# microhh/rte-rrtmgp-cpp

Hardware: AMD Instinct MI355X
Metric: columns/sec (LW+SW full solve, 140 lay x 256 gpt) (higher is better)
Workload: dtype f64; 1 GPU; C4 synthetic 16384 columns/GPU (16384 in total) x 140 layers x 256 g-points, LW+SW clear-sky, RCEMIP profile, synthetic k-distribution (real shapes); columns_per_gpu=16384, columns_total=16384, nlay=140, ngpt=256, flux_mode=broadband (do_broadband solvers, g-point sums on chip), columns_sorted=False, parallelism=columns sharded x1, all-gather of broadband fluxes

## Files before the change

rte-rrtmgp-cpp_amd/csrc/rrx_common.h:

```cpp
#ifndef RRX_COMMON_H
#define RRX_COMMON_H

#include <hip/hip_runtime.h>
#include <cfloat>
#include <cstdlib>
#include <cmath>
#include <string>
#include <vector>
#include <stdexcept>
#include <type_traits>

typedef signed char Bool;

namespace rrx
{
    struct Tuning
    {
        int lw_variant = 0;
        int sw_variant = 0;
        int bb_min_groups = 512;
        int bb_gsplit = 0;
        int sync_waves = 1;
        int go_share = 1;
        int go_window = 1;
    };
    Tuning& tuning();

    void set_error(const std::string& msg);
    int check_launch(const char* what);

    constexpr int WAVE = 64;

    template<typename F> struct Lim;
    template<> struct Lim<double>
    {
        __host__ __device__ static constexpr double eps() { return DBL_EPSILON; }
        __host__ __device__ static constexpr double tiny() { return DBL_MIN; }
        __host__ __device__ static constexpr double k_min() { return 1.e-12; }
    };
    template<> struct Lim<float>
    {
        __host__ __device__ static constexpr float eps() { return FLT_EPSILON; }
        __host__ __device__ static constexpr float tiny() { return FLT_MIN; }
        __host__ __device__ static constexpr float k_min() { return 1.e-4f; }
    };

    __device__ __forceinline__ float shfl(const float v, const int src_lane) { return __shfl(v, src_lane, WAVE); }
    __device__ __forceinline__ double shfl(const double v, const int src_lane) { return __shfl(v, src_lane, WAVE); }

#ifndef RRX_NT_LOADS
#define RRX_NT_LOADS 0
#endif
#ifndef RRX_NT_STORES
#define RRX_NT_STORES 0
#endif
    template<typename F, int V> struct Vec { F v[V]; };

    template<typename F, int V>
    __device__ __forceinline__ Vec<F,V> load_cols(const F* __restrict__ p)
    {
        Vec<F,V> r;
        if constexpr (V == 1)
        {
#if RRX_NT_LOADS
            r.v[0] = __builtin_nontemporal_load(p);
#else
            r.v[0] = p[0];
#endif
        }
        else
        {
            typedef F vecT __attribute__((ext_vector_type(V)));
#if RRX_NT_LOADS
            const vecT t = __builtin_nontemporal_load(reinterpret_cast<const vecT*>(p));
#else
            const vecT t = *reinterpret_cast<const vecT*>(p);
#endif
            #pragma unroll
            for (int i=0; i<V; ++i) r.v[i] = t[i];
        }
        return r;
    }

    template<typename F, int V>
    __device__ __forceinline__ void store_cols(F* __restrict__ p, const Vec<F,V>& r)
    {
        if constexpr (V == 1)
        {
#if RRX_NT_STORES
            __builtin_nontemporal_store(r.v[0], p);
#else
            p[0] = r.v[0];
#endif
        }
        else
        {
            typedef F vecT __attribute__((ext_vector_type(V)));
            vecT t;
            #pragma unroll
            for (int i=0; i<V; ++i) t[i] = r.v[i];
#if RRX_NT_STORES
            __builtin_nontemporal_store(t, reinterpret_cast<vecT*>(p));
#else
            *reinterpret_cast<vecT*>(p) = t;
#endif
        }
    }

    template<typename F>
    __device__ __forceinline__ void add_rounded(F& acc, const F x)
    {
        #pragma clang fp contract(off)
        acc = acc + x;
    }

    __device__ __forceinline__ double fast_rcp(const double x)
    {
        double r = __builtin_amdgcn_rcp(x);
        double e = fma(-x, r, 1.0); r = fma(r, e, r);
        e = fma(-x, r, 1.0); r = fma(r, e, r);
        return r;
    }
#ifndef RRX_F32_IEEE_RCP
    __device__ __forceinline__ float fast_rcp(const float x)
    {
        float r = __builtin_amdgcn_rcpf(x);
        const float e = fmaf(-x, r, 1.0f); r = fmaf(r, e, r);
        return r;
    }
#else
    __device__ __forceinline__ float fast_rcp(const float x) { return 1.0f / x; }
#endif

    __device__ __forceinline__ double exp_neg(const double x)
    {
        const double n = __builtin_rint(x * 0x1.71547652b82fep+0);
        double r = fma(n, -0x1.62e42f0000000p-1, x);
        r = fma(n, -0x1.df473de6af279p-26, r);
        double p = 0x1.af389ecfc4b9cp-26;
        p = fma(p, r, 0x1.28917c89a43a7p-22); p = fma(p, r, 0x1.71de0db2f6b19p-19); p = fma(p, r, 0x1.a019b9149a41cp-16);
        p = fma(p, r, 0x1.a01a01a7c2efep-13); p = fma(p, r, 0x1.6c16c17889ef1p-10); p = fma(p, r, 0x1.11111111109b5p-7);
        p = fma(p, r, 0x1.5555555553d68p-5); p = fma(p, r, 0x1.5555555555556p-3); p = fma(p, r, 0x1.0000000000001p-1);
        const double t = fma(r*r, p, r);
        return __builtin_amdgcn_ldexp(t + 1.0, (int)n);
    }
    static __device__ const double exp2_64_table[64] = {
        0x1.0000000000000p+0, 0x1.02c9a3e778061p+0, 0x1.059b0d3158574p+0, 0x1.0874518759bc8p+0, 0x1.0b5586cf9890fp+0, 0x1.0e3ec32d3d1a2p+0,
        0x1.11301d0125b51p+0, 0x1.1429aaea92de0p+0, 0x1.172b83c7d517bp+0, 0x1.1a35beb6fcb75p+0, 0x1.1d4873168b9aap+0, 0x1.2063b88628cd6p+0,
        0x1.2387a6e756238p+0, 0x1.26b4565e27cddp+0, 0x1.29e9df51fdee1p+0, 0x1.2d285a6e4030bp+0, 0x1.306fe0a31b715p+0, 0x1.33c08b26416ffp+0,
        0x1.371a7373aa9cbp+0, 0x1.3a7db34e59ff7p+0, 0x1.3dea64c123422p+0, 0x1.4160a21f72e2ap+0, 0x1.44e086061892dp+0, 0x1.486a2b5c13cd0p+0,
        0x1.4bfdad5362a27p+0, 0x1.4f9b2769d2ca7p+0, 0x1.5342b569d4f82p+0, 0x1.56f4736b527dap+0, 0x1.5ab07dd485429p+0, 0x1.5e76f15ad2148p+0,
        0x1.6247eb03a5585p+0, 0x1.6623882552225p+0, 0x1.6a09e667f3bcdp+0, 0x1.6dfb23c651a2fp+0, 0x1.71f75e8ec5f74p+0, 0x1.75feb564267c9p+0,
        0x1.7a11473eb0187p+0, 0x1.7e2f336cf4e62p+0, 0x1.82589994cce13p+0, 0x1.868d99b4492edp+0, 0x1.8ace5422aa0dbp+0, 0x1.8f1ae99157736p+0,
        0x1.93737b0cdc5e5p+0, 0x1.97d829fde4e50p+0, 0x1.9c49182a3f090p+0, 0x1.a0c667b5de565p+0, 0x1.a5503b23e255dp+0, 0x1.a9e6b5579fdbfp+0,
        0x1.ae89f995ad3adp+0, 0x1.b33a2b84f15fbp+0, 0x1.b7f76f2fb5e47p+0, 0x1.bcc1e904bc1d2p+0, 0x1.c199bdd85529cp+0, 0x1.c67f12e57d14bp+0,
        0x1.cb720dcef9069p+0, 0x1.d072d4a07897cp+0, 0x1.d5818dcfba487p+0, 0x1.da9e603db3285p+0, 0x1.dfc97337b9b5fp+0, 0x1.e502ee78b3ff6p+0,
        0x1.ea4afa2a490dap+0, 0x1.efa1bee615a27p+0, 0x1.f50765b6e4540p+0, 0x1.fa7c1819e90d8p+0};
    __device__ __forceinline__ void exp_table_fill(double* lds_table)
    {
        if (threadIdx.x < 64) lds_table[threadIdx.x] = exp2_64_table[threadIdx.x];
    }
    __device__ __forceinline__ double exp_neg(const double x, const double* lds_table)
    {
        const double magic = 0x1.8p+52;
        const double t = fma(x, 0x1.71547652b82fep+6, magic);
        const double nf = t - magic;
// ... 204 lines not shown
```

rte-rrtmgp-cpp_amd/csrc/rrx_solver_lw.hip:

```cpp
#include "rrx_common.h"
#include "rrx_hip.h"

#pragma clang fp contract(fast)

namespace
{
using namespace rrx;

constexpr int CL = 8;
constexpr int LL = 8;

template<typename F, int V, int K, bool JAC, bool ACC>
__global__ void __launch_bounds__(256, 2)
lw_noscat_scan_kernel(
        const int ncol, const int nlay, const int ngpt, const int top_at_1, const int imu,
        const F* __restrict__ secants, const F* __restrict__ weights,
        const F* __restrict__ tau, const F* __restrict__ lay_source, const F* __restrict__ lev_source,
        const F* __restrict__ sfc_emis, const F* __restrict__ sfc_src, const F* __restrict__ inc_flux,
        F* __restrict__ flux_up, F* __restrict__ flux_dn,
        const F* __restrict__ sfc_src_jac, F* __restrict__ flux_up_jac, const int sync_waves)
{
    constexpr int W = 2;
    const int lane = threadIdx.x & 63;
    const int wave = threadIdx.x >> 6;
// ... 179 lines not shown
    {
        F dn[V];
        #pragma unroll
        for (int v=0; v<V; ++v) dn[v] = dn_in[v];
        #pragma unroll
        for (int j=0; j<K; ++j)
        {
            Vec<F,V> o;
            #pragma unroll
            for (int v=0; v<V; ++v) { o.v[v] = scale * dn[v]; dn[v] = tr[j][v]*dn[v] + sdn[j][v]; }
            put(flux_dn, j, o);
        }
    }
    {
        F up[V], jc[V];
        #pragma unroll
        for (int v=0; v<V; ++v) { up[v] = up_in[v]; jc[v] = JAC ? jac_in[v] : F(0.); }
        #pragma unroll
        for (int j=K-1; j>=0; --j)
        {
            Vec<F,V> o, oj;
            #pragma unroll
            for (int v=0; v<V; ++v)
            {
                up[v] = tr[j][v]*up[v] + sup[j][v];
                o.v[v] = scale * up[v];
                if constexpr (JAC) { jc[v] = tr[j][v]*jc[v]; oj.v[v] = scale * jc[v]; }
            }
            put(flux_up, j, o);
            if constexpr (JAC) put(flux_up_jac, j, oj);
        }
    }
    }
}


#ifndef RRX_LW_LACC
#define RRX_LW_LACC 1
#endif
#ifndef RRX_LW_EXP_TABLE
#define RRX_LW_EXP_TABLE 1
#endif
#ifndef RRX_LW_TIMING
#define RRX_LW_TIMING 0
#endif
#if RRX_LW_TIMING
__device__ unsigned long long g_lw_clk[16][8];
#define RRX_LW_T(k) { const unsigned long long t_ = __builtin_readcyclecounter(); lw_acc[k] += t_ - lw_t; lw_t = t_; }
#else
#define RRX_LW_T(k)
#endif
#ifndef RRX_LW_LACC32
#define RRX_LW_LACC32 1
#endif
#ifndef RRX_LW_EV
#define RRX_LW_EV 1
#endif
#ifndef RRX_LW_F32_WAVES
#define RRX_LW_F32_WAVES 2
#endif
template<typename F, int V, int K, int W, int CLT, bool LITE, bool GS = false, int EV = RRX_LW_EV, int NW = (W > 4 ? W : 4), bool BND = false,
         bool JAC = false, bool MU = false, bool OPT = false>
__global__ void __launch_bounds__(64*NW, (NW > W) ? RRX_LW_F32_WAVES : (NW > 4 ? 1 : 2))
lw_noscat_bb_kernel(
        const int ncol, const int nlay, const int ngpt, const int top_at_1,
        const F* __restrict__ secants, const F* __restrict__ weights,
        const F* __restrict__ tau, const F* __restrict__ lay_source , const F* __restrict__ lev_source,
        const F* __restrict__ blay, const F* __restrict__ blev, const int* __restrict__ gpoint_bands,
        const F* __restrict__ sfc_emis, const F* __restrict__ sfc_src, const F* __restrict__ inc_flux,
        F* __restrict__ flux_up, F* __restrict__ flux_dn, const int gper, const size_t part_stride,
        const int* __restrict__ band_lims, const F* __restrict__ sfc_src_jac = nullptr, F* __restrict__ flux_up_jac = nullptr,
        const int nmus = 1, const F* __restrict__ opt_fit = nullptr, F* __restrict__ secants_out = nullptr)
{
    static_assert(!(GS && BND), "a by-band launch is its own g-point split");
    static_assert(!(JAC && BND), "no by-band Jacobian");
    static_assert(!MU || (LITE && !BND), "several angles: Planck-lite inputs, no by-band form");
    static_assert(!OPT || (LITE && !BND), "optimal angles: Planck-lite inputs, no by-band form");
    static_assert(!(OPT && MU), "optimal angles are one quadrature angle");
    const int g_lo = BND ? max(band_lims[2*blockIdx.y] - 1, 0) : (GS ? blockIdx.y*gper : 0);
    const int g_hi = BND ? min(band_lims[2*blockIdx.y+1], ngpt) : (GS ? min(ngpt, g_lo + gper) : ngpt);
    if constexpr (GS || BND) { flux_up += blockIdx.y*part_stride; flux_dn += blockIdx.y*part_stride; }
    if constexpr (GS && JAC) flux_up_jac += blockIdx.y*part_stride;
    constexpr int CL = CLT, LL = 64/CLT;
    const int tid = threadIdx.x, lane = tid & 63, wave = tid >> 6;
    const int cl = lane & (CL-1), ll = lane / CL;
    const int h = wave % W, w0 = wave - h;
    const int bx = ((NW/W)*CL*V*sizeof(F) < 128) ? xcd_contiguous(blockIdx.x, gridDim.x) : int(blockIdx.x);
    const int wave_col0 = (bx*(NW/W) + wave/W) * (CL*V);
    __shared__ F xch[4*V][NW][CL];
    __shared__ F xsum[OPT ? V : 1][NW][CL];
    __shared__ F lds_b[LITE ? (2*K+1)*V : 1][64*NW];
    constexpr bool ETAB = sizeof(F) == 8 && RRX_LW_EXP_TABLE;
    __shared__ F lds_etab[ETAB ? 64 : 1];
    if constexpr (ETAB) { exp_table_fill(lds_etab); __syncthreads(); }
    int icol = wave_col0 + cl*V;
    const bool active = icol < ncol;
    if (!active) icol = (wave_col0 < ncol) ? wave_col0 : 0;
    const bool writer = active && wave_col0 < ncol;
    const int nlev = nlay + 1;
    const size_t ncl = size_t(ncol);
    const int t0 = (h*LL + ll)*K;
    const F pi = F(3.14159265358979323846);
    const F tau_thres = sqrt(sqrt(Lim<F>::eps()));

    constexpr bool LACC = RRX_LW_LACC && ((sizeof(F) == 8 && V == 1) || (sizeof(F) == 4 && V == 2 && RRX_LW_LACC32));
    __shared__ F lds_acc[LACC ? 2*K*V : 1][64*NW];
    F acc_up[LACC ? 1 : K][V], acc_dn[LACC ? 1 : K][V];
    #pragma unroll
    for (int j=0; j<K; ++j)
        #pragma unroll
        for (int v=0; v<V; ++v)
        {
            if constexpr (LACC) { lds_acc[j*V+v][tid] = F(0.); lds_acc[(K+j)*V+v][tid] = F(0.); }
            else { acc_up[j][v] = F(0.); acc_dn[j][v] = F(0.); }
        }
    F acc_jc[JAC ? K : 1][V];
    if constexpr (JAC)
    {
        #pragma unroll
        for (int j=0; j<K; ++j)
            #pragma unroll
            for (int v=0; v<V; ++v) acc_jc[j][v] = F(0.);
    }

    auto lay_off = [&](const int j) -> unsigned
    {
        const int sc = min(max(t0 + j, 0), nlay-1);
        return unsigned(top_at_1 ? sc : nlay-1-sc)*unsigned(ncol) + unsigned(icol);
    };
    auto lev_off = [&](const int j) -> unsigned
    {
        const int tc = min(t0 + j, nlay);
        return unsigned(top_at_1 ? tc : nlay-tc)*unsigned(ncol) + unsigned(icol);
    };

    struct Loads { Vec<F,V> a0[K], a1[K], a2[LITE ? 1 : K], x_next, x_prev, emis, ssrc, D, inc; };
    auto issue = [&](const int g, Loads& L, Vec<F,V>& J)
    {
        const F* __restrict__ t_g = tau + size_t(g)*ncl*nlay;
        const F* __restrict__ l_g = lay_source + size_t(g)*ncl*nlay;
        #pragma unroll
        for (int j=0; j<K; ++j) { const unsigned o = lay_off(j); L.a0[j] = load_cols<F,V>(t_g + o); L.a1[j] = load_cols<F,V>(l_g + o); }
        if constexpr (!LITE)
        {
            const F* __restrict__ v_g = lev_source + size_t(g)*ncl*nlev;
            #pragma unroll
            for (int j=0; j<K; ++j) L.a2[j] = load_cols<F,V>(v_g + lev_off(j));
            L.x_next = load_cols<F,V>(v_g + lev_off(K));
        }
        else
        {
            L.x_next = load_cols<F,V>(l_g + lay_off(K));
            L.x_prev = load_cols<F,V>(l_g + lay_off(-1));
        }
        const size_t sfc = size_t(g)*ncl + icol;
        L.emis = load_cols<F,V>(sfc_emis + sfc); L.ssrc = load_cols<F,V>(sfc_src + sfc);
        if constexpr (!MU && !OPT) L.D = load_cols<F,V>(secants + sfc);
        if (inc_flux != nullptr) L.inc = load_cols<F,V>(inc_flux + sfc);
        if constexpr (JAC) J = load_cols<F,V>(sfc_src_jac + sfc);
    };

    Loads nxt;
    Vec<F,V> jnxt, jcur;
    if (!BND || g_lo < g_hi) issue(g_lo, nxt, jnxt);
    int cur_bnd = -1;
    const F wgt = weights[0];
    const F scale = pi * wgt;
    Vec<F,V> d_next, c_emis, c_ssrc, c_inc;
    F scale_mu;
    if constexpr (MU) d_next = load_cols<F,V>(secants + size_t(g_lo)*ncl + icol);
    F fit1 = F(0.), fit2 = F(0.);

#if RRX_LW_TIMING
    unsigned long long lw_acc[8] = {0, 0, 0, 0, 0, 0, 0, 0}, lw_t = __builtin_readcyclecounter();
#endif
    for (int igpt=g_lo; igpt<g_hi; ++igpt)
    {
    RRX_LW_T(7)
    std::conditional_t<MU, Loads&, Loads> cur = nxt;
    if constexpr (JAC) jcur = jnxt;
    if constexpr (MU) { c_emis = cur.emis; c_ssrc = cur.ssrc; c_inc = cur.inc; }

    if constexpr (LITE)
    {
        const int ib = gpoint_bands[igpt] - 1;
        if (ib != cur_bnd)
        {
            cur_bnd = ib;
            const F* __restrict__ bl = blay + size_t(ib)*ncl*nlay;
            const F* __restrict__ bv = blev + size_t(ib)*ncl*nlev;
            #pragma unroll
            for (int j=0; j<K; ++j)
            {
                const Vec<F,V> x = load_cols<F,V>(bl + lay_off(j));
                #pragma unroll
                for (int v=0; v<V; ++v) lds_b[j*V+v][tid] = x.v[v];
            }
            #pragma unroll
            for (int j=0; j<=K; ++j)
            {
                const Vec<F,V> x = load_cols<F,V>(bv + lev_off(j));
                #pragma unroll
                for (int v=0; v<V; ++v) lds_b[(K+j)*V+v][tid] = x.v[v];
            }
            if constexpr (OPT) { fit1 = opt_fit[2*ib]; fit2 = opt_fit[2*ib+1]; }
        }
    }

    if constexpr (OPT)
    {
        F s[V];
        #pragma unroll
        for (int v=0; v<V; ++v) s[v] = F(0.);
        #pragma unroll
        for (int j=0; j<K; ++j)
        {
            const bool valid = (t0 + j) < nlay;
            #pragma unroll
            for (int v=0; v<V; ++v) s[v] += valid ? cur.a0[j].v[v] : F(0.);
        }
        #pragma unroll
        for (int d=1; d<LL; d<<=1)
            #pragma unroll
            for (int v=0; v<V; ++v) s[v] += shfl(s[v], lane ^ (d*CL));
        if (ll == 0)
        {
            #pragma unroll
            for (int v=0; v<V; ++v) xsum[v][wave][cl] = s[v];
        }
        RRX_LW_T(4)
        __syncthreads();
        #pragma unroll
        for (int v=0; v<V; ++v)
        {
            F t = F(0.);
            #pragma unroll
            for (int w=0; w<W; ++w) t += xsum[v][w0+w][cl];
            F e;
            if constexpr (ETAB) e = exp_neg(-t, lds_etab); else e = exp_neg(-t);
            cur.D.v[v] = fit1*e + fit2;
// ... 18 lines not shown
    do
    {
    if constexpr (MU)
    {
        cur.D = d_next;
        scale_mu = pi * weights[imu];
        const bool last = imu == nmus-1;
        d_next = load_cols<F,V>(secants + (size_t(last ? 0 : imu + 1)*ngpt + (last ? min(igpt + 1, g_hi - 1) : igpt))*ncl + icol);
        #pragma unroll
        for (int j=0; j<K; ++j)
            #pragma unroll
            for (int v=0; v<V; ++v) asm volatile("" : "+v"(cur.a1[j].v[v]));
        #pragma unroll
        for (int v=0; v<V; ++v) asm volatile("" : "+v"(cur.x_prev.v[v]), "+v"(cur.x_next.v[v]));
    }
    F tr[K][V], sdn[K][V], sup[K][V];
    F A[V], Bdn[V], Bup[V], lva[V];
    #pragma unroll
    for (int v=0; v<V; ++v) { A[v] = F(1.); Bdn[v] = F(0.); Bup[v] = F(0.); lva[v] = level_src(0, v); }
    #pragma unroll
    for (int j=0; j<K; ++j)
    {
        const bool valid = (t0 + j) < nlay;
        #pragma unroll
        for (int v=0; v<V; ++v)
        {
            F tvj = cur.a0[j].v[v];
            const int e = j*V + v - EV*V;
            if (e >= 0) asm volatile("" : "+v"(tvj) : "v"(sup[e / V][e % V]));
            const F lvb = level_src(j+1, v);
            F lsj = cur.a1[j].v[v];
            if constexpr (LITE) lsj *= lds_b[j*V+v][tid];
            const F tau_loc = (valid ? tvj : F(0.)) * cur.D.v[v];
            F trans;
            if constexpr (ETAB) trans = exp_neg(-tau_loc, lds_etab); else trans = exp_neg(-tau_loc);
            const F fact = tau_loc > tau_thres ? (F(1.) - trans) * fast_rcp(tau_loc) - trans
                                               : tau_loc * (F(.5) + tau_loc * (F(-1./3.) + tau_loc * F(1./8.)));
            const F omt = F(1.) - trans;
            const F s_dn = omt * lvb + F(2.) * fact * (lsj - lvb);
            const F s_up = omt * lva[v] + F(2.) * fact * (lsj - lva[v]);
            lva[v] = lvb;
            tr[j][v] = trans; sdn[j][v] = s_dn; sup[j][v] = s_up;
            Bdn[v] = tr[j][v]*Bdn[v] + sdn[j][v];
            Bup[v] += A[v]*sup[j][v];
            A[v] *= tr[j][v];
        }
    }

    RRX_LW_T(0)
    F dn_in[V], up_in[V], jc_in[V];
    #pragma unroll
    for (int v=0; v<V; ++v)
    {
        F a = A[v], b = Bdn[v];
        #pragma unroll
        for (int d=1; d<LL; d<<=1)
        {
            const F a2 = shfl(a, lane - d*CL), b2 = shfl(b, lane - d*CL);
            if (ll >= d) { b = a*b2 + b; a = a*a2; }
        }
        F xa = F(1.), xb = F(0.);
        if (ll == LL-1) { xch[4*v+0][wave][cl] = a; xch[4*v+1][wave][cl] = b; }
        RRX_LW_T(1)
        __syncthreads();
        RRX_LW_T(6)
        if (v == 0) if (!MU || imu == nmus-1)
        {
            __builtin_amdgcn_sched_barrier(0);
            issue(min(igpt + 1, g_hi - 1), nxt, jnxt);
            __builtin_amdgcn_sched_barrier(0);
        }
        F fa = F(1.), fb = F(0.);
        #pragma unroll
        for (int w=0; w<W; ++w)
        {
            const F oa = xch[4*v+0][w0+w][cl], ob = xch[4*v+1][w0+w][cl];
            if (w == h) { xa = fa; xb = fb; }
            fb = oa*fb + ob; fa = oa*fa;
        }
        if (h > 0) { b = a*xb + b; a = a*xa; }
        F ae = shfl(a, lane - CL), be = shfl(b, lane - CL);
        if (ll == 0) { ae = xa; be = xb; }
        const F dn_top = (inc_flux != nullptr) ? (MU ? c_inc : cur.inc).v[v] / pi : F(0.);
        dn_in[v] = ae*dn_top + be;
        const F dn_sfc = fa*dn_top + fb;
        const F up_sfc = dn_sfc * (F(1.) - (MU ? c_emis : cur.emis).v[v]) + (MU ? c_emis : cur.emis).v[v] * (MU ? c_ssrc : cur.ssrc).v[v];

        a = A[v]; b = Bup[v];
        #pragma unroll
        for (int d=1; d<LL; d<<=1)
        {
            const F a2 = shfl(a, lane + d*CL), b2 = shfl(b, lane + d*CL);
            if (ll + d < LL) { b = a*b2 + b; a = a*a2; }
        }
        xa = F(1.); xb = F(0.);
        if (ll == 0) { xch[4*v+2][wave][cl] = a; xch[4*v+3][wave][cl] = b; }
        RRX_LW_T(2)
        __syncthreads();
        RRX_LW_T(6)
        #pragma unroll
        for (int w=W-1; w>=1; --w)
            if (w > h) { const F oa = xch[4*v+2][w0+w][cl], ob = xch[4*v+3][w0+w][cl]; xb = oa*xb + ob; xa = oa*xa; }
        if (h < W-1) { b = a*xb + b; a = a*xa; }
        ae = shfl(a, lane + CL); be = shfl(b, lane + CL);
        if (ll == LL-1) { ae = xa; be = xb; }
        up_in[v] = ae*up_sfc + be;
        if constexpr (JAC) jc_in[v] = ae * (MU ? c_emis : cur.emis).v[v] * jcur.v[v];
    }

    #pragma unroll
    for (int v=0; v<V; ++v)
    {
        F dn = dn_in[v];
        #pragma unroll
        for (int j=0; j<K; ++j)
        {
            if constexpr (LACC) { F a = lds_acc[(K+j)*V+v][tid]; add_rounded(a, (MU ? scale_mu : scale)*dn); lds_acc[(K+j)*V+v][tid] = a; }
            else add_rounded(acc_dn[j][v], (MU ? scale_mu : scale)*dn);
            dn = tr[j][v]*dn + sdn[j][v];
        }
        F up = up_in[v];
        #pragma unroll
        for (int j=K-1; j>=0; --j)
        {
            up = tr[j][v]*up + sup[j][v];
            if constexpr (LACC) { F a = lds_acc[j*V+v][tid]; add_rounded(a, (MU ? scale_mu : scale)*up); lds_acc[j*V+v][tid] = a; }
            else add_rounded(acc_up[j][v], (MU ? scale_mu : scale)*up);
        }
        if constexpr (JAC)
        {
            F jc = jc_in[v];
            #pragma unroll
            for (int j=K-1; j>=0; --j) { jc = tr[j][v]*jc; add_rounded(acc_jc[j][v], (MU ? scale_mu : scale)*jc); }
        }
    }
    RRX_LW_T(3)
    } while (MU && ++imu < nmus);
    }
#if RRX_LW_TIMING
    if (lane == 0) for (int k=0; k<8; ++k) atomicAdd(&g_lw_clk[wave & 15][k], lw_acc[k]);
#endif

    if (!writer) return;
    #pragma unroll
    for (int j=0; j<K; ++j)
    {
        const int t = t0 + j;
        if (t <= nlay)
        {
            const size_t o = size_t(icol) + size_t(top_at_1 ? t : nlay - t)*ncl;
            Vec<F,V> u, d;
            #pragma unroll
            for (int v=0; v<V; ++v)
            {
                if constexpr (LACC) { u.v[v] = lds_acc[j*V+v][tid]; d.v[v] = lds_acc[(K+j)*V+v][tid]; }
                else { u.v[v] = acc_up[j][v]; d.v[v] = acc_dn[j][v]; }
            }
            store_cols<F,V>(flux_up + o, u);
            store_cols<F,V>(flux_dn + o, d);
            if constexpr (JAC)
// ... 126 lines not shown
    else if (optimal_angle_fit == nullptr) bad = "optimal_angle_fit is null";
    else if (tau == nullptr) bad = "tau is null";
    else if (secants == nullptr) bad = "secants is null";
    if (bad != nullptr) { set_error(std::string(entry) + ": " + bad); return 1; }
    RRX_TRY
    lw_optimal_secants_kernel<F><<<dim3(ceil_div(ncol, 256), ngpt), 256, 0, static_cast<hipStream_t>(stream)>>>(
            ncol, nlay, gpoint_bands, optimal_angle_fit, tau, secants);
    RRX_CATCH(entry)
}

template<typename F, int V>
bool launch_scan(
        hipStream_t st, const bool jac, const bool acc,
        const int ncol, const int nlay, const int ngpt, const int top_at_1, const int imu,
        const F* secants, const F* weights, const F* tau, const F* lay_source, const F* lev_source,
        const F* sfc_emis, const F* sfc_src, const F* inc_flux, F* flux_up, F* flux_dn,
        const F* sfc_src_jac, F* flux_up_jac)
{
    const dim3 grid(ceil_div(ncol, 2*CL*V), ngpt);
    const int sync_waves = tuning().sync_waves;
    return with_k<2, 4, 6, 9, 12, 17>(ceil_div(nlay+1, 2*LL), [&](auto kk)
    {
        with_flag(jac, [&](auto j) { with_flag(acc, [&](auto a)
        {
            lw_noscat_scan_kernel<F,V,decltype(kk)::value,decltype(j)::value,decltype(a)::value><<<grid, 256, 0, st>>>(
                ncol, nlay, ngpt, top_at_1, imu, secants, weights, tau, lay_source, lev_source,
                sfc_emis, sfc_src, inc_flux, flux_up, flux_dn, sfc_src_jac, flux_up_jac, sync_waves);
        }); });
    });
}

template<typename F>
struct BbArgs
{
    int ncol, nlay, ngpt, top_at_1;
    const F *secants, *weights, *tau, *lay_source , *lev_source, *blay, *blev;
    const int* gpoint_bands;
    const F *sfc_emis, *sfc_src, *inc_flux;
    F *flux_up, *flux_dn;
    const int* band_lims; int nbnd;
    const F* sfc_src_jac; F* flux_up_jac;
    int nmus;
    const F* opt_fit = nullptr; F* secants_out = nullptr;
};

template<typename F, int V, int W, int CLT, bool LITE, int NW, bool JAC, bool MU, bool OPT = false>
bool launch_bb2(hipStream_t st, const BbArgs<F>& a)
{
    static_assert(!MU || LITE, "several angles: Planck-lite inputs only");
    static_assert(!OPT || (LITE && !MU), "optimal angles: Planck-lite inputs, one angle");
    if (size_t(a.ncol)*(a.nlay+1) >= (size_t(1) << 31)) return false;
    const int groups = ceil_div(a.ncol, (NW/W)*CLT*V);
    const int need = ceil_div(a.nlay+1, (64/CLT)*W);
    if (need > ((CLT == 16 || W == 8) ? 9 : 5)) return false;
    auto with_tiling_k = [&](auto launch)
    {
        if constexpr (CLT == 16) return with_k<2, 4, 6, 9>(need, launch);
        else if constexpr (W == 8) return with_k<5, 7, 9>(need, launch);
        else return with_k<2, 3, 5>(need, launch);
    };
    const size_t nlevcol = size_t(a.ncol)*(a.nlay+1);
    if (!JAC && !MU && !OPT && a.band_lims != nullptr)
    {
        if constexpr (LITE)
        {
            const dim3 grid(groups, a.nbnd);
            return with_tiling_k([&](auto kk)
            {
                lw_noscat_bb_kernel<F,V,decltype(kk)::value,W,CLT,LITE,false,RRX_LW_EV,NW,true><<<grid, 64*NW, 0, st>>>(
                    a.ncol, a.nlay, a.ngpt, a.top_at_1, a.secants, a.weights, a.tau, a.lay_source, a.lev_source, a.blay, a.blev,
                    a.gpoint_bands, a.sfc_emis, a.sfc_src, a.inc_flux, a.flux_up, a.flux_dn, 0, nlevcol, a.band_lims);
            });
        }
        return false;
    }
    const int gper = ceil_div(a.ngpt, broadband_gsplit(groups, a.ngpt, (NW > 4) ? 256 : 512));
    const int nsplit = ceil_div(a.ngpt, gper);
    constexpr int NARR = JAC ? 3 : 2;
    StreamScratch scratch(st);
    F* out_up = a.flux_up; F* out_dn = a.flux_dn; F* out_jc = a.flux_up_jac;
    if (nsplit > 1)
    {
        out_up = scratch.get<F>(NARR*nsplit*nlevcol); out_dn = out_up + nsplit*nlevcol;
        if (JAC) out_jc = out_dn + nsplit*nlevcol;
    }
    const dim3 grid(groups, nsplit);
    with_tiling_k([&](auto kk) { with_flag(nsplit > 1, [&](auto gs)
    {
        lw_noscat_bb_kernel<F,V,decltype(kk)::value,W,CLT,LITE,decltype(gs)::value,RRX_LW_EV,NW,false,JAC,MU,OPT><<<grid, 64*NW, 0, st>>>(
            a.ncol, a.nlay, a.ngpt, a.top_at_1, a.secants, a.weights, a.tau, a.lay_source, a.lev_source, a.blay, a.blev,
            a.gpoint_bands, a.sfc_emis, a.sfc_src, a.inc_flux, out_up, out_dn, gper, nlevcol, nullptr, a.sfc_src_jac, out_jc,
            MU ? a.nmus : 1, OPT ? a.opt_fit : nullptr, OPT ? a.secants_out : nullptr);
    }); });
    if (nsplit > 1)
        sum_ranges_kernel<F,NARR><<<dim3(ceil_div(nlevcol, 256), NARR), 256, 0, st>>>(nlevcol, nsplit, out_up, a.flux_up, a.flux_dn,
                                                                                      a.flux_up_jac);
    return true;
}

template<typename F, bool LITE, bool JAC = false, bool MU = false, bool OPT = false>
bool lw_fused_broadband(
        hipStream_t st, const int ncol, const int nlay, const int ngpt, const int top_at_1,
        const F* secants, const F* weights, const F* tau, const F* lay_source, const F* lev_source,
        const F* blay, const F* blev, const int* gpoint_bands,
        const F* sfc_emis, const F* sfc_src, const F* inc_flux, F* flux_up, F* flux_dn,
        const int* band_lims = nullptr, const int nbnd = 0 ,
        const F* sfc_src_jac = nullptr, F* flux_up_jac = nullptr, const int nmus = 1,
        const F* opt_fit = nullptr, F* secants_out = nullptr)
{
    const BbArgs<F> a{ncol, nlay, ngpt, top_at_1, secants, weights, tau, lay_source, lev_source, blay, blev, gpoint_bands,
                      sfc_emis, sfc_src, inc_flux, flux_up, flux_dn, band_lims, nbnd, sfc_src_jac, flux_up_jac, nmus,
                      opt_fit, secants_out};
    if constexpr (sizeof(F) == 8)
    {
        if (launch_bb2<F,1,4,16,LITE,4,JAC,MU,OPT>(st, a)) return true;
        if (launch_bb2<F,1,8,16,LITE,8,JAC,MU,OPT>(st, a)) return true;
        return launch_bb2<F,1,8,8,LITE,8,JAC,MU,OPT>(st, a);
    }
    else
    {
        if (tuning().lw_variant == 15 && launch_bb2<F,1,4,16,LITE,8,JAC,MU,OPT>(st, a)) return true;
        if (ncol % 2 == 0 && launch_bb2<F,2,4,16,LITE,4,JAC,MU,OPT>(st, a)) return true;
        if (ncol % 4 == 0 && launch_bb2<F,4,4,8,LITE,4,JAC,MU,OPT>(st, a)) return true;
        if (ncol % 2 == 0 && launch_bb2<F,2,8,16,LITE,8,JAC,MU,OPT>(st, a)) return true;
        if (ncol % 2 == 0 && launch_bb2<F,2,8,8,LITE,8,JAC,MU,OPT>(st, a)) return true;
        return launch_bb2<F,1,4,16,LITE,8,JAC,MU,OPT>(st, a);
    }
}

bool lw_fused_allowed()
{
    const int v = tuning().lw_variant;
    return v != 1 && v != 7;
}

#define RRX_LW_ARGS_CALL ncol, nlay, ngpt, top_at_1, imu, secants, weights, tau, lay_source, lev_source, \
        sfc_emis, sfc_src, inc_flux, up, dn, sfc_src_jac, flux_up_jac

template<typename F>
int lw_solver_noscat_impl(
        const int ncol, const int nlay, const int ngpt, const Bool top_at_1, const int nmus,
        const F* secants, const F* weights,
        const F* tau, const F* lay_source, const F* lev_source,
        const F* sfc_emis, const F* sfc_src, const F* inc_flux,
        F* flux_up, F* flux_dn,
        const Bool do_broadband, F* flux_up_loc, F* flux_dn_loc,
        const Bool do_jacobians, const F* sfc_src_jac, F* flux_up_jac,
        void* stream)
{
    RRX_TRY
    hipStream_t st = static_cast<hipStream_t>(stream);
    if (ncol <= 0 || nlay <= 0 || ngpt <= 0) throw std::runtime_error("empty problem");
    if (nmus < 1 || nmus > 4) throw std::runtime_error("n_quad_angs must be 1..4");
    if (do_broadband && (flux_up_loc == nullptr || flux_dn_loc == nullptr)) throw std::runtime_error("do_broadband needs flux_*_loc");
    const bool jac = do_jacobians && sfc_src_jac != nullptr && flux_up_jac != nullptr;
    const int variant = tuning().lw_variant;

    if (do_broadband && !jac && nmus == 1 && lw_fused_allowed() &&
        lw_fused_broadband<F,false>(st, ncol, nlay, ngpt, top_at_1, secants, weights, tau, lay_source, lev_source,
                                    (const F*)nullptr, (const F*)nullptr, (const int*)nullptr, sfc_emis, sfc_src, inc_flux,
                                    flux_up_loc, flux_dn_loc))
        return 0;

    F* up = flux_up; F* dn = flux_dn;
    WorkspaceLease lease(st);
    const size_t nlevcol = size_t(ncol)*(nlay+1);
    if (do_broadband) { up = lease.get<F>(2*nlevcol*ngpt); dn = up + nlevcol*ngpt; }
// ... 261 lines not shown
    if (flux_net != nullptr) flux_net[i] -= d;
}

template<typename F>
int lw_flux_up_adjust_impl(const int ncol, const int nlev, const F* flux_up_jac, const F* t_sfc_old, const F* t_sfc_new,
                           F* flux_up, F* flux_net, void* stream)
{
    RRX_TRY
    if (ncol <= 0 || nlev <= 0) throw std::runtime_error("empty problem");
    if (flux_up_jac == nullptr) throw std::runtime_error("flux_up_jac is null");
    if (t_sfc_old == nullptr || t_sfc_new == nullptr) throw std::runtime_error("surface temperatures missing");
    if (flux_up == nullptr) throw std::runtime_error("flux_up is null");
    const size_t n = size_t(ncol)*nlev;
    lw_flux_up_adjust_kernel<F><<<ceil_div(n, 256), 256, 0, static_cast<hipStream_t>(stream)>>>(n, ncol, flux_up_jac, t_sfc_old, t_sfc_new,
                                                                                                 flux_up, flux_net);
    RRX_CATCH("rrx_lw_flux_up_adjust")
}

template<typename F>
int lw_solver_noscat_fractions_byband_impl(
        const int ncol, const int nlay, const int ngpt, const int nbnd, const Bool top_at_1,
        const F* secants, const F* weights, const F* tau, const F* pfrac, const F* blay, const F* blev, const int* gpoint_bands,
        const int* band_lims, const F* sfc_emis, const F* sfc_src, const F* inc_flux,
        F* bnd_up, F* bnd_dn, F* bnd_net, F* flux_up, F* flux_dn, void* stream)
{
    RRX_TRY
    hipStream_t st = static_cast<hipStream_t>(stream);
    check_byband_args(ncol, nlay, ngpt, nbnd, band_lims);
    if (gpoint_bands == nullptr) throw std::runtime_error("gpoint_bands is null");
    if (bnd_up == nullptr || bnd_dn == nullptr) throw std::runtime_error("band flux outputs missing");
    const size_t nlevcol = size_t(ncol)*(nlay+1);
    const bool fused = lw_fused_allowed() &&
        lw_fused_broadband<F,true>(st, ncol, nlay, ngpt, top_at_1, secants, weights, tau, pfrac, (const F*)nullptr,
                                   blay, blev, gpoint_bands, sfc_emis, sfc_src, inc_flux, bnd_up, bnd_dn, band_lims, nbnd);
    if (!fused)
    {
        WorkspaceLease lease(st);
        const F* ws = lw_fractions_per_gpoint<F>(lease, ncol, nlay, ngpt, top_at_1, secants, weights, tau, pfrac, blay, blev,
                                                 gpoint_bands, sfc_emis, sfc_src, inc_flux, (const F*)nullptr, stream);
        if (ws == nullptr) return 1;
        sum_bands_kernel<F><<<dim3(ceil_div(nlevcol, 256), nbnd, 2), 256, 0, st>>>(nlevcol, ngpt, band_lims, ws, bnd_up, bnd_dn,
                                                                                      (F*)nullptr);
    }
    launch_byband_outputs<F,2>(st, nlevcol, nbnd, bnd_up, bnd_dn, (const F*)nullptr, bnd_net, flux_up, flux_dn, (F*)nullptr);
    RRX_CATCH("rrx_lw_solver_noscat_fractions_byband")
}
}


extern "C"
{
int rrx_set_lw_variant(int v)
{
    if (v != 0 && v != 1 && v != 4 && v != 7 && v != 15)
    {
        rrx::set_error("rrx_set_lw_variant: " + std::to_string(v) + " is not an LW variant; accepted: 0 (default), 1 (serial kernel), "
                       "4 (general kernel with 64-B rows), 7 (no one-kernel broadband form), 15 (fp32: one column per lane in the "
                       "one-kernel broadband form)");
        return 1;
    }
    rrx::tuning().lw_variant = v;
    return 0;
}
#if RRX_LW_TIMING
int rrx_lw_timing(unsigned long long* out)
{
    unsigned long long zero[16*8] = {0};
    if (hipDeviceSynchronize() != hipSuccess || hipMemcpyFromSymbol(out, HIP_SYMBOL(g_lw_clk), 16*8*sizeof(unsigned long long)) != hipSuccess) return 1;
    return hipMemcpyToSymbol(HIP_SYMBOL(g_lw_clk), zero, sizeof(zero)) == hipSuccess ? 0 : 1;
}
#endif

int rrx_lw_secants_array_f64(int ncol, int ngpt, int n_gauss_quad, int max_gauss_pts, const double* gauss_Ds, double* secants, void* stream)
{
    RRX_TRY
    lw_secants_array_kernel<double><<<rrx::ceil_div(size_t(ncol)*ngpt*n_gauss_quad, 256), 256, 0, static_cast<hipStream_t>(stream)>>>(
            ncol, ngpt, n_gauss_quad, max_gauss_pts, gauss_Ds, secants);
    RRX_CATCH("rrx_lw_secants_array")
}

int rrx_lw_secants_array_f32(int ncol, int ngpt, int n_gauss_quad, int max_gauss_pts, const float* gauss_Ds, float* secants, void* stream)
{
    RRX_TRY
    lw_secants_array_kernel<float><<<rrx::ceil_div(size_t(ncol)*ngpt*n_gauss_quad, 256), 256, 0, static_cast<hipStream_t>(stream)>>>(
            ncol, ngpt, n_gauss_quad, max_gauss_pts, gauss_Ds, secants);
    RRX_CATCH("rrx_lw_secants_array")
}

int rrx_lw_solver_noscat_f64(
        int ncol, int nlay, int ngpt, Bool top_at_1, int nmus,
        const double* secants, const double* weights,
        const double* tau, const double* lay_source, const double* lev_source,
        const double* sfc_emis, const double* sfc_src, const double* inc_flux,
        double* flux_up, double* flux_dn,
        Bool do_broadband, double* flux_up_loc, double* flux_dn_loc,
        Bool do_jacobians, const double* sfc_src_jac, double* flux_up_jac, void* stream)
{
    return lw_solver_noscat_impl<double>(ncol, nlay, ngpt, top_at_1, nmus, secants, weights, tau, lay_source, lev_source,
            sfc_emis, sfc_src, inc_flux, flux_up, flux_dn, do_broadband, flux_up_loc, flux_dn_loc,
            do_jacobians, sfc_src_jac, flux_up_jac, stream);
}

int rrx_lw_solver_noscat_f32(
        int ncol, int nlay, int ngpt, Bool top_at_1, int nmus,
        const float* secants, const float* weights,
        const float* tau, const float* lay_source, const float* lev_source,
        const float* sfc_emis, const float* sfc_src, const float* inc_flux,
        float* flux_up, float* flux_dn,
        Bool do_broadband, float* flux_up_loc, float* flux_dn_loc,
        Bool do_jacobians, const float* sfc_src_jac, float* flux_up_jac, void* stream)
{
// ... 64 lines not shown
```

Measured before the change: 1.426 million columns/s.

## Add one-wave-per-column-group fp64 LW broadband scan using DPP and shuffles

Adds a W=1 geometry of the LW broadband kernel in which each wave holds a whole column group (4 column lanes by 16 level lanes). The cross-wave LDS exchange and its two __syncthreads per g-point are replaced by in-row DPP shifts plus cross-row shuffles for the up and down linear-recurrence scans. This geometry becomes the first fp64 choice for plain Planck-lite launches, with variant 14 to fall back to the old form. Each lane now covers more levels (larger K), which raises register pressure, and the waves of a workgroup drift apart without barriers, which may hurt cache sharing.

```diff
diff --git a/rte-rrtmgp-cpp_amd/csrc/rrx_common.h b/rte-rrtmgp-cpp_amd/csrc/rrx_common.h
--- a/rte-rrtmgp-cpp_amd/csrc/rrx_common.h
+++ b/rte-rrtmgp-cpp_amd/csrc/rrx_common.h
@@ -48,6 +48,21 @@
     __device__ __forceinline__ float shfl(const float v, const int src_lane) { return __shfl(v, src_lane, WAVE); }
     __device__ __forceinline__ double shfl(const double v, const int src_lane) { return __shfl(v, src_lane, WAVE); }
 
+    template<int CTRL>
+    __device__ __forceinline__ float dpp_row(const float v, const float fill)
+    {
+        return __int_as_float(__builtin_amdgcn_update_dpp(__float_as_int(fill), __float_as_int(v), CTRL, 0xf, 0xf, false));
+    }
+    template<int CTRL>
+    __device__ __forceinline__ double dpp_row(const double v, const double fill)
+    {
+        const int lo = __builtin_amdgcn_update_dpp(__double2loint(fill), __double2loint(v), CTRL, 0xf, 0xf, false);
+        const int hi = __builtin_amdgcn_update_dpp(__double2hiint(fill), __double2hiint(v), CTRL, 0xf, 0xf, false);
+        return __hiloint2double(hi, lo);
+    }
+    template<int N, typename F> __device__ __forceinline__ F row_shr(const F v, const F fill) { return dpp_row<0x110 + N>(v, fill); }
+    template<int N, typename F> __device__ __forceinline__ F row_shl(const F v, const F fill) { return dpp_row<0x100 + N>(v, fill); }
+
 #ifndef RRX_NT_LOADS
 #define RRX_NT_LOADS 0
 #endif
@@ -112,6 +127,13 @@
     {
         #pragma clang fp contract(off)
         acc = acc + x;
+    }
+
+    template<typename F>
+    __device__ __forceinline__ F mul_rounded(const F x, const F y)
+    {
+        #pragma clang fp contract(off)
+        return x * y;
     }
 
     __device__ __forceinline__ double fast_rcp(const double x)
diff --git a/rte-rrtmgp-cpp_amd/csrc/rrx_solver_lw.hip b/rte-rrtmgp-cpp_amd/csrc/rrx_solver_lw.hip
--- a/rte-rrtmgp-cpp_amd/csrc/rrx_solver_lw.hip
+++ b/rte-rrtmgp-cpp_amd/csrc/rrx_solver_lw.hip
@@ -255,6 +255,9 @@
 #endif
 #ifndef RRX_LW_LACC32
 #define RRX_LW_LACC32 1
+#endif
+#ifndef RRX_LW_WAVE_ALIGN
+#define RRX_LW_WAVE_ALIGN 0
 #endif
 #ifndef RRX_LW_EV
 #define RRX_LW_EV 1
@@ -280,6 +283,9 @@
     static_assert(!MU || (LITE && !BND), "several angles: Planck-lite inputs, no by-band form");
     static_assert(!OPT || (LITE && !BND), "optimal angles: Planck-lite inputs, no by-band form");
     static_assert(!(OPT && MU), "optimal angles are one quadrature angle");
+    constexpr bool ONE = (W == 1);
+    static_assert(!ONE || (CLT == 4 && NW == 4), "one wave per column group: 4 column-lanes x 16 level-lanes, four groups per workgroup");
+    static_assert(!(ONE && OPT), "optimal angles: the W > 1 geometries");
     const int g_lo = BND ? max(band_lims[2*blockIdx.y] - 1, 0) : (GS ? blockIdx.y*gper : 0);
     const int g_hi = BND ? min(band_lims[2*blockIdx.y+1], ngpt) : (GS ? min(ngpt, g_lo + gper) : ngpt);
     if constexpr (GS || BND) { flux_up += blockIdx.y*part_stride; flux_dn += blockIdx.y*part_stride; }
@@ -290,7 +296,7 @@
     const int h = wave % W, w0 = wave - h;
     const int bx = ((NW/W)*CL*V*sizeof(F) < 128) ? xcd_contiguous(blockIdx.x, gridDim.x) : int(blockIdx.x);
     const int wave_col0 = (bx*(NW/W) + wave/W) * (CL*V);
-    __shared__ F xch[4*V][NW][CL];
+    __shared__ F xch[ONE ? 1 : 4*V][ONE ? 1 : NW][CL];
     __shared__ F xsum[OPT ? V : 1][NW][CL];
     __shared__ F lds_b[LITE ? (2*K+1)*V : 1][64*NW];
     constexpr bool ETAB = sizeof(F) == 8 && RRX_LW_EXP_TABLE;
@@ -389,6 +395,9 @@
         const int ib = gpoint_bands[igpt] - 1;
         if (ib != cur_bnd)
         {
+#if RRX_LW_WAVE_ALIGN
+            if constexpr (ONE) __syncthreads();
+#endif
             cur_bnd = ib;
             const F* __restrict__ bl = blay + size_t(ib)*ncl*nlay;
             const F* __restrict__ bv = blev + size_t(ib)*ncl*nlev;
@@ -513,60 +522,120 @@
     #pragma unroll
     for (int v=0; v<V; ++v)
     {
-        F a = A[v], b = Bdn[v];
-        #pragma unroll
-        for (int d=1; d<LL; d<<=1)
-        {
-            const F a2 = shfl(a, lane - d*CL), b2 = shfl(b, lane - d*CL);
-            if (ll >= d) { b = a*b2 + b; a = a*a2; }
-        }
-        F xa = F(1.), xb = F(0.);
-        if (ll == LL-1) { xch[4*v+0][wave][cl] = a; xch[4*v+1][wave][cl] = b; }
-        RRX_LW_T(1)
-        __syncthreads();
-        RRX_LW_T(6)
-        if (v == 0) if (!MU || imu == nmus-1)
-        {
-            __builtin_amdgcn_sched_barrier(0);
-            issue(min(igpt + 1, g_hi - 1), nxt, jnxt);
-            __builtin_amdgcn_sched_barrier(0);
-        }
-        F fa = F(1.), fb = F(0.);
-        #pragma unroll
-        for (int w=0; w<W; ++w)
-        {
-            const F oa = xch[4*v+0][w0+w][cl], ob = xch[4*v+1][w0+w][cl];
-            if (w == h) { xa = fa; xb = fb; }
-            fb = oa*fb + ob; fa = oa*fa;
-        }
-        if (h > 0) { b = a*xb + b; a = a*xa; }
-        F ae = shfl(a, lane - CL), be = shfl(b, lane - CL);
-        if (ll == 0) { ae = xa; be = xb; }
-        const F dn_top = (inc_flux != nullptr) ? (MU ? c_inc : cur.inc).v[v] / pi : F(0.);
-        dn_in[v] = ae*dn_top + be;
-        const F dn_sfc = fa*dn_top + fb;
-        const F up_sfc = dn_sfc * (F(1.) - (MU ? c_emis : cur.emis).v[v]) + (MU ? c_emis : cur.emis).v[v] * (MU ? c_ssrc : cur.ssrc).v[v];
-
-        a = A[v]; b = Bup[v];
-        #pragma unroll
-        for (int d=1; d<LL; d<<=1)
-        {
-            const F a2 = shfl(a, lane + d*CL), b2 = shfl(b, lane + d*CL);
-            if (ll + d < LL) { b = a*b2 + b; a = a*a2; }
-        }
-        xa = F(1.); xb = F(0.);
-        if (ll == 0) { xch[4*v+2][wave][cl] = a; xch[4*v+3][wave][cl] = b; }
-        RRX_LW_T(2)
-        __syncthreads();
-        RRX_LW_T(6)
-        #pragma unroll
-        for (int w=W-1; w>=1; --w)
-            if (w > h) { const F oa = xch[4*v+2][w0+w][cl], ob = xch[4*v+3][w0+w][cl]; xb = oa*xb + ob; xa = oa*xa; }
-        if (h < W-1) { b = a*xb + b; a = a*xa; }
-        ae = shfl(a, lane + CL); be = shfl(b, lane + CL);
-        if (ll == LL-1) { ae = xa; be = xb; }
-        up_in[v] = ae*up_sfc + be;
-        if constexpr (JAC) jc_in[v] = ae * (MU ? c_emis : cur.emis).v[v] * jcur.v[v];
+        if constexpr (ONE)
+        {
+            const int q = lane >> 4;
+            F a = A[v], b = Bdn[v];
+            {
+                const F a2 = row_shr<CL>(a, F(1.)), b2 = row_shr<CL>(b, F(0.));
+                b = a*b2 + b; a = a*a2;
+            }
+            {
+                const F a2 = row_shr<2*CL>(a, F(1.)), b2 = row_shr<2*CL>(b, F(0.));
+                b = a*b2 + b; a = a*a2;
+            }
+            RRX_LW_T(1)
+            if (v == 0) if (!MU || imu == nmus-1)
+            {
+                __builtin_amdgcn_sched_barrier(0);
+                issue(min(igpt + 1, g_hi - 1), nxt, jnxt);
+                __builtin_amdgcn_sched_barrier(0);
+            }
+            const int up1 = (lane | (16-CL)) - 16;
+            F t1a = shfl(a, up1), t1b = shfl(b, up1);
+            if (q < 1) { t1a = F(1.); t1b = F(0.); }
+            const F ja = a*t1a, jb = a*t1b + b;
+            F t2a = shfl(ja, up1 - 16), t2b = shfl(jb, up1 - 16);
+            if (q < 2) { t2a = F(1.); t2b = F(0.); }
+            const F pb = t1a*t2b + t1b, pa = t1a*t2a;
+            const F ea = row_shr<CL>(a, F(1.)), eb = row_shr<CL>(b, F(0.));
+            const F dn_top = (inc_flux != nullptr) ? (MU ? c_inc : cur.inc).v[v] / pi : F(0.);
+            dn_in[v] = (ea*pa)*dn_top + (ea*pb + eb);
+            const F fb = a*pb + b, fa = a*pa;
+            const F dn_sfc = fa*dn_top + fb;
+            const F emis_v = (MU ? c_emis : cur.emis).v[v];
+            const F ssrc_v = (MU ? c_ssrc : cur.ssrc).v[v];
+            const F up_sfc = shfl(fma(dn_sfc, F(1.) - emis_v, mul_rounded(emis_v, ssrc_v)), 64 - CL + cl);
+
+            a = A[v]; b = Bup[v];
+            {
+                const F a2 = row_shl<CL>(a, F(1.)), b2 = row_shl<CL>(b, F(0.));
+                b = a*b2 + b; a = a*a2;
+            }
+            {
+                const F a2 = row_shl<2*CL>(a, F(1.)), b2 = row_shl<2*CL>(b, F(0.));
+                b = a*b2 + b; a = a*a2;
+            }
+            const int dn1 = (lane & ~(16-CL)) + 16;
+            F u1a = shfl(a, dn1), u1b = shfl(b, dn1);
+            if (q > 2) { u1a = F(1.); u1b = F(0.); }
+            const F ka = a*u1a, kb = a*u1b + b;
+            F u2a = shfl(ka, dn1 + 16), u2b = shfl(kb, dn1 + 16);
+            if (q > 1) { u2a = F(1.); u2b = F(0.); }
+            const F xb = u1a*u2b + u1b, xa = u1a*u2a;
+            const F ga = row_shl<CL>(a, F(1.)), gb = row_shl<CL>(b, F(0.));
+            const F ae = ga*xa;
+            up_in[v] = ae*up_sfc + (ga*xb + gb);
+            if constexpr (JAC) jc_in[v] = ae * emis_v * jcur.v[v];
+            RRX_LW_T(2)
+        }
+        else
+        {
+            F a = A[v], b = Bdn[v];
+            #pragma unroll
+            for (int d=1; d<LL; d<<=1)
+            {
+                const F a2 = shfl(a, lane - d*CL), b2 = shfl(b, lane - d*CL);
+                if (ll >= d) { b = a*b2 + b; a = a*a2; }
+            }
+            F xa = F(1.), xb = F(0.);
+            if (ll == LL-1) { xch[4*v+0][wave][cl] = a; xch[4*v+1][wave][cl] = b; }
+            RRX_LW_T(1)
+            __syncthreads();
+            RRX_LW_T(6)
+            if (v == 0) if (!MU || imu == nmus-1)
+            {
+                __builtin_amdgcn_sched_barrier(0);
+                issue(min(igpt + 1, g_hi - 1), nxt, jnxt);
+                __builtin_amdgcn_sched_barrier(0);
+            }
+            F fa = F(1.), fb = F(0.);
+            #pragma unroll
+            for (int w=0; w<W; ++w)
+            {
+                const F oa = xch[4*v+0][w0+w][cl], ob = xch[4*v+1][w0+w][cl];
+                if (w == h) { xa = fa; xb = fb; }
+                fb = oa*fb + ob; fa = oa*fa;
+            }
+            if (h > 0) { b = a*xb + b; a = a*xa; }
+            F ae = shfl(a, lane - CL), be = shfl(b, lane - CL);
+            if (ll == 0) { ae = xa; be = xb; }
+            const F dn_top = (inc_flux != nullptr) ? (MU ? c_inc : cur.inc).v[v] / pi : F(0.);
+            dn_in[v] = ae*dn_top + be;
+            const F dn_sfc = fa*dn_top + fb;
+            const F up_sfc = dn_sfc * (F(1.) - (MU ? c_emis : cur.emis).v[v]) + (MU ? c_emis : cur.emis).v[v] * (MU ? c_ssrc : cur.ssrc).v[v];
+
+            a = A[v]; b = Bup[v];
+            #pragma unroll
+            for (int d=1; d<LL; d<<=1)
+            {
+                const F a2 = shfl(a, lane + d*CL), b2 = shfl(b, lane + d*CL);
+                if (ll + d < LL) { b = a*b2 + b; a = a*a2; }
+            }
+            xa = F(1.); xb = F(0.);
+            if (ll == 0) { xch[4*v+2][wave][cl] = a; xch[4*v+3][wave][cl] = b; }
+            RRX_LW_T(2)
+            __syncthreads();
+            RRX_LW_T(6)
+            #pragma unroll
+            for (int w=W-1; w>=1; --w)
+                if (w > h) { const F oa = xch[4*v+2][w0+w][cl], ob = xch[4*v+3][w0+w][cl]; xb = oa*xb + ob; xa = oa*xa; }
+            if (h < W-1) { b = a*xb + b; a = a*xa; }
+            ae = shfl(a, lane + CL); be = shfl(b, lane + CL);
+            if (ll == LL-1) { ae = xa; be = xb; }
+            up_in[v] = ae*up_sfc + be;
+            if constexpr (JAC) jc_in[v] = ae * (MU ? c_emis : cur.emis).v[v] * jcur.v[v];
+        }
     }
 
     #pragma unroll
@@ -799,17 +868,17 @@
     if (size_t(a.ncol)*(a.nlay+1) >= (size_t(1) << 31)) return false;
     const int groups = ceil_div(a.ncol, (NW/W)*CLT*V);
     const int need = ceil_div(a.nlay+1, (64/CLT)*W);
-    if (need > ((CLT == 16 || W == 8) ? 9 : 5)) return false;
+    if (need > ((CLT == 16 || W == 8 || W == 1) ? 9 : 5)) return false;
     auto with_tiling_k = [&](auto launch)
     {
-        if constexpr (CLT == 16) return with_k<2, 4, 6, 9>(need, launch);
+        if constexpr (CLT == 16 || W == 1) return with_k<2, 4, 6, 9>(need, launch);
         else if constexpr (W == 8) return with_k<5, 7, 9>(need, launch);
         else return with_k<2, 3, 5>(need, launch);
     };
     const size_t nlevcol = size_t(a.ncol)*(a.nlay+1);
     if (!JAC && !MU && !OPT && a.band_lims != nullptr)
     {
-        if constexpr (LITE)
+        if constexpr (LITE && W > 1)
         {
             const dim3 grid(groups, a.nbnd);
             return with_tiling_k([&](auto kk)
@@ -860,6 +929,8 @@
                       opt_fit, secants_out};
     if constexpr (sizeof(F) == 8)
     {
+        if constexpr (LITE && !JAC && !MU && !OPT)
+            if (band_lims == nullptr && tuning().lw_variant != 14 && launch_bb2<F,1,1,4,LITE,4,false,false,false>(st, a)) return true;
         if (launch_bb2<F,1,4,16,LITE,4,JAC,MU,OPT>(st, a)) return true;
         if (launch_bb2<F,1,8,16,LITE,8,JAC,MU,OPT>(st, a)) return true;
         return launch_bb2<F,1,8,8,LITE,8,JAC,MU,OPT>(st, a);
@@ -1227,11 +1298,11 @@
 {
 int rrx_set_lw_variant(int v)
 {
-    if (v != 0 && v != 1 && v != 4 && v != 7 && v != 15)
+    if (v != 0 && v != 1 && v != 4 && v != 7 && v != 14 && v != 15)
     {
         rrx::set_error("rrx_set_lw_variant: " + std::to_string(v) + " is not an LW variant; accepted: 0 (default), 1 (serial kernel), "
-                       "4 (general kernel with 64-B rows), 7 (no one-kernel broadband form), 15 (fp32: one column per lane in the "
-                       "one-kernel broadband form)");
+                       "4 (general kernel with 64-B rows), 7 (no one-kernel broadband form), 14 (fp64: four waves per column group in the "
+                       "plain one-kernel broadband form), 15 (fp32: one column per lane in the one-kernel broadband form)");
         return 1;
     }
     rrx::tuning().lw_variant = v;
```

Result: slower. 1.229 million columns/s (-13.9%).
